# askerlee/segtran

Hardware: AMD Instinct MI355X
Metric: train-step images/sec (cfg2, re-associated op order) (higher is better)
Workload: dtype f32; 1 GPU; REFUGE fundus 2D, segtran eff-b4, translayers 3, layercompress 1,1,2,2, 512x512, bs 6/GPU; global_batch=6, per_gpu_batch=6, parallelism=dp1, step=fwd+BCE/Dice+bwd+allreduce+clip+BertAdam, op_order=re-associated, ranks=1

## Files before the change

### include/segx.h

```cpp
#ifndef SEGX_H
#define SEGX_H
#include <stdint.h>
#ifdef __cplusplus
extern "C" {
#endif

int segx_version(void);
int segx_last_error(char* buf, int buflen);

enum { SEGX_EPI_NONE = 0, SEGX_EPI_GELU = 1 ,
       SEGX_EPI_SWISH = 2  };
enum { SEGX_BIAS_NONE = 0, SEGX_BIAS_N = 1 , SEGX_BIAS_M = 2  };
enum { SEGX_ENGINE_F32 = 0, SEGX_ENGINE_BF16X6 = 1 };
enum { SEGX_ENGINE_SEL_DEFAULT = 0, SEGX_ENGINE_SEL_F32 = 1, SEGX_ENGINE_SEL_BF16X6 = 2 };
enum { SEGX_TILE_AUTO = 0, SEGX_TILE_128x128 = 1, SEGX_TILE_64x64 = 2, SEGX_TILE_128x32 = 3, SEGX_TILE_32x128 = 4, SEGX_TILE_64x128 = 5,
       SEGX_TILE_256x128 = 6, SEGX_TILE_WS128x128 = 7, SEGX_TILE_WS128x256 = 8, SEGX_TILE_WS64x256 = 9,
       SEGX_TILE_WS96x256 = 10, SEGX_TILE_WS256x96 = 11,
       SEGX_TILE_SKINNY_NT = 12   };
typedef struct {
    int32_t M, N, K, nb0, nb1;
    int64_t a_b0, a_b1, a_m, a_k;
    int64_t b_b0, b_b1, b_n, b_k;
    int64_t c_b0, c_b1, c_m;
    float alpha;
// ... 74 lines not shown
int segx_seg_loss_fwd(const float* logits, const float* mask, const float* pos_weight, const float* class_w, float* out,
                      float* ws, int B, int C, int64_t S, float dice_w, void* stream);
int segx_seg_loss_bwd(const float* logits, const float* mask, const float* pos_weight, const float* class_w, const float* ws,
                      const float* grad_out, float* dlogits, int B, int C, int64_t S, float dice_w, void* stream);
int segx_mt_bertadam_step(void* const* params, const void* const* grads, void* const* m, void* const* v, const int64_t* sizes,
                          const int* chunk_tensor, const int64_t* chunk_off, const int* chunk_first, const int* active,
                          const float* lr, const float* wd, int ntensors, int nchunks, int chunk,
                          float max_global_norm, float max_tensor_norm, float sched, float b1, float b2, float eps,
                          float* ws, void* stream);

int segx_mt_gather(const void* const* src, void* const* dst, const int64_t* sizes, const int* chunk_tensor, const int64_t* chunk_off,
                   int chunk_begin, int nchunks, int chunk, void* stream);

int64_t segx_bn_ws_floats(int B, int C, int64_t S);
int segx_bn_act_bwd_reduce(const float* dY, const float* X, const float* mean, const float* var, const float* w, const float* b,
                           float* dw, float* db, float* ws, int B, int C, int64_t S, float eps, int act,
                           const float* gate, const float* dpool, float inv_S, float dc_p, uint64_t seed, uint64_t offset, void* stream);
int segx_bn_act_bwd_apply(const float* dY, const float* X, const float* mean, const float* var, const float* w, const float* b,
                          const float* sum_dw, const float* sum_db, float* dX, int B, int C, int64_t S, float eps, int act,
                          float inv_n, const float* gate, const float* dpool, float inv_S, float dc_p, uint64_t seed, uint64_t offset, void* stream);
int64_t segx_plane_chunks(int64_t S);
int64_t segx_bn_pool_chunks(int B, int64_t S, int auto_stats);
int64_t segx_bn_parts_floats(int B, int C, int64_t S);
int segx_bn_stats_local(const float* X, float* part, float* ws, int B, int C, int64_t S, void* stream);
int segx_bn_act_fwd2(const float* X, const float* parts, int nparts, float* mean, float* var, float* run_mean, float* run_var, float momentum,
                     const float* w, const float* b, float* Y, float* psum, const float* resid, float dc_p, uint64_t seed, uint64_t offset,
                     int B, int C, int64_t S, float eps, int act, int64_t parts_floats, int64_t y_bs, void* stream);
int segx_team_status(int clear);
int segx_team_cap(void);
int segx_occupy(int wgs, int heavy, float ms, float* sink, void* stream);
int segx_bn_act_bwd2(const float* dY, const float* X, const float* mean, const float* var, const float* w, const float* b,
                     float* dX, float* dw, float* db, float* ws, int B, int C, int64_t S, float eps, int act, int training,
                     const float* gate, const float* dpool, float inv_S, float dc_p, uint64_t seed, uint64_t offset, int64_t dy_bs, int64_t ws_floats, void* stream);
int segx_se_fwd2(const float* psum, int nch, float inv_S, const float* W1, const float* b1, const float* W2, const float* b2, const float* Wproj,
                 float* p, float* hpre, float* gate, float* Wb, int B, int C, int Cs, int M, void* stream);
int64_t segx_se_ws2_floats(int B, int C, int Cs);
int segx_se_bwd2(const float* dWb, const float* Wproj, const float* dgate, const float* gate, const float* hpre, const float* p, const float* W1,
                 const float* W2, float inv_S, float* dpool, float* dW1, float* db1, float* dW2, float* db2, float* dWproj, float* ws,
                 int B, int C, int Cs, int M, void* stream);
int segx_dwconv2d_fwd(const float* X, const float* W, float* Y, int B, int C, int H, int Wd, int OH, int OW, int k, int stride,
                      int pad_t, int pad_l, void* stream);
int64_t segx_dwconv2d_pool_chunks(int OH, int OW);
int segx_dwconv2d_bias_act_pool(const float* X, const float* W, const float* bias, float* Y, float* psum, int B, int C, int H, int Wd, int OH, int OW,
                                int k, int stride, int pad_t, int pad_l, int act, void* stream);
int segx_dwconv2d_bwd_data(const float* dY, const float* W, float* dX, int B, int C, int H, int Wd, int OH, int OW, int k,
                           int stride, int pad_t, int pad_l, void* stream);
int64_t segx_dwconv2d_wgrad_rows(int OH, int OW);
int64_t segx_dwconv2d_bwd_fused_rows(int H, int Wd, int OH, int OW, int k, int stride, int pad_t, int pad_l);
int segx_dwconv2d_bwd_fused(const float* dY, const float* X, const float* W, float* dX, float* part, int B, int C, int H, int Wd, int OH, int OW,
                            int k, int stride, int pad_t, int pad_l, void* stream);
int segx_dwconv2d_bwd_weight_direct(const float* dY, const float* X, float* dW, int B, int C, int H, int Wd, int OH, int OW, int k,
                                    int stride, int pad_t, int pad_l, void* stream);
int segx_dwconv2d_bwd_weight(const float* dY, const float* X, float* part, int B, int C, int H, int Wd, int OH, int OW, int k,
                             int stride, int pad_t, int pad_l, void* stream);
int segx_plane_scale(const float* X, const float* gate, float* Y, int64_t planes, int64_t S, void* stream);
int segx_plane_bias_add(const float* X, const float* bias, float* Y, int64_t planes, int C, int64_t S, void* stream);
int segx_plane_dot(const float* A, const float* Bm, float* out, int64_t planes, int64_t S, void* stream);

int64_t segx_gn_ws_floats(int B, int C, int G);
int segx_groupnorm_fwd(const float* X, const float* w, const float* b, float* Y, float* mean, float* rstd, float* ws,
                       int B, int C, int G, int64_t S, float eps, void* stream);
int segx_groupnorm_bwd(const float* dY, const float* X, const float* w, const float* mean, const float* rstd, float* dX,
                       float* dw, float* db, float* ws, int B, int C, int G, int64_t S, float* plane_dx_sums, void* stream);
int64_t segx_interp_gn_nparts(int64_t float4_per_plane, int cpg);
int segx_interp_linear_fwd_axis2_gn(const float* in, const float* base, float* out, int64_t outer, int n1_in, int n1_out, int n2_in, int n2_out,
                                    int64_t inner, int cpg, float* parts, int nparts, void* stream);
// ... 117 lines not shown
```

### segtran_amd/csrc/backbone.hip

```cpp
#include "common.h"
#include <mutex>
#include <unordered_map>

namespace segx {

enum { ACT_NONE = 0, ACT_SWISH = 1, ACT_RELU = 2, ACT_LEAKY = 3  };

__device__ __forceinline__ float sigm(float x) { return 1.0f / (1.0f + __expf(-x)); }
__device__ __forceinline__ float act_fwd(float u, int act) {
    return act == ACT_SWISH ? u * sigm(u) : act == ACT_RELU ? fmaxf(u, 0.f) : act == ACT_LEAKY ? (u > 0.f ? u : 0.2f * u) : u;
}
__device__ __forceinline__ float act_grad(float u, int act) {
    if (act == ACT_SWISH) { const float s = sigm(u); return s * (1.0f + u * (1.0f - s)); }
    if (act == ACT_RELU) return u > 0.f ? 1.0f : 0.f;
    if (act == ACT_LEAKY) return u > 0.f ? 1.0f : 0.2f;
    return 1.0f;
}

__device__ __forceinline__ float drop_connect_scale(float p, uint64_t seed, uint64_t offset, const uint64_t* __restrict__ rbase, int sample) {
    if (!(p > 0.f)) return 1.0f;
    return dropout_scale(seed, 0, offset + (rbase ? *rbase : 0) + (uint64_t)sample, p, 1.0f / (1.0f - p));
}
__device__ __forceinline__ void bn_fold_sums(const float* __restrict__ ws, int c, int nparts, float& a, float& q) {
    const int lane = threadIdx.x & 63;
// ... 1313 lines not shown
        float a = 0.f;
#pragma unroll 16
        for (int i = 0; i < n; ++i) a += dz[i] * W2[(int64_t)(k0 + i) * Cs + j];
        part[((int64_t)b * gridDim.x + blockIdx.x) * Cs + j] = a;
    }
}
__global__ __launch_bounds__(256) void se_wgrad_all_kernel(const float* __restrict__ dz2, const float* __restrict__ dhpre, const float* __restrict__ p,
                                                           const float* __restrict__ hpre, float* __restrict__ dW1, float* __restrict__ db1,
                                                           float* __restrict__ dW2, float* __restrict__ db2, const float* __restrict__ dWb,
                                                           const float* __restrict__ gate, float* __restrict__ dW, int B, int C, int Cs, int64_t MK) {
    const int64_t idx = (int64_t)blockIdx.x * 256 + threadIdx.x, n1 = (int64_t)C * Cs;
    if (idx < n1) {
        const int c = (int)(idx / Cs), j = (int)(idx % Cs);
        float a1 = 0.f, a2 = 0.f, s1 = 0.f, s2 = 0.f;
        for (int b = 0; b < B; ++b) {
            const float hp = hpre[(int64_t)b * Cs + j], dz = dz2[(int64_t)b * C + c], dh = dhpre[(int64_t)b * Cs + j];
            a2 += dz * (hp * sigm(hp)); a1 += dh * p[(int64_t)b * C + c]; s2 += dz; s1 += dh;
        }
        dW2[(int64_t)c * Cs + j] = a2; dW1[(int64_t)j * C + c] = a1;
        if (j == 0) db2[c] = s2;
        if (c == 0) db1[j] = s1;
        return;
    }
    const int64_t i = idx - n1;
    if (!dWb || i >= MK) return;
    const int k = (int)(i % C);
    float s = 0.f;
    for (int b = 0; b < B; ++b) s += dWb[(int64_t)b * MK + i] * gate[(int64_t)b * C + k];
    dW[i] = s;
}

static inline int plane_chunks(int64_t S, int per_thread) { return (int)i64max(1, i64min(64, (S + 256 * per_thread - 1) / (256 * per_thread))); }

}

using namespace segx;
#define SEGX_STREAM hipStream_t stream = (hipStream_t)stream_

static inline int64_t bn_team_floats(int B, int C, int64_t S, bool backward) {
    int kp = 0;
    if (S <= 0 || bn_auto_form(B, S, backward, &kp) != 1) return 0;
    return (int64_t)C * B * bn_team_chunks(S, kp) * (TEAM_SLOT + TEAM_MBOX);
}
template <int LDS_FLOATS>
__global__ __launch_bounds__(256) void occupy_kernel(unsigned long long ticks, float* sink) {
    __shared__ float hold[LDS_FLOATS];
    const unsigned long long t0 = wall_clock64();
    float acc = 0.f;
    while (wall_clock64() - t0 < ticks) { acc += hold[threadIdx.x & 15]; __builtin_amdgcn_s_sleep(32); }
    if (sink && acc == 12345.678f) sink[0] = acc;
}
extern "C" int segx_occupy(int wgs, int heavy, float ms, float* sink, void* stream_) {
    SEGX_STREAM; SEGX_REQUIRE(wgs > 0 && wgs <= 65535 && ms >= 0.f && ms <= 2000.f, "segx_occupy: bad args");
    const unsigned long long ticks = (unsigned long long)(ms * 1e5f);
    if (heavy) hipLaunchKernelGGL((occupy_kernel<20 * 1024>), dim3(wgs), dim3(256), 0, stream, ticks, sink);
    else hipLaunchKernelGGL((occupy_kernel<16>), dim3(wgs), dim3(256), 0, stream, ticks, sink);
    return check_launch("segx_occupy");
}
extern "C" int segx_team_status(int clear) {
    const TeamHost& h = team_host();
    const unsigned n = __atomic_load_n(h.host, __ATOMIC_RELAXED);
    if (clear && n) __atomic_fetch_sub(h.host, n, __ATOMIC_RELAXED);
    return (int)(n > 0x7fffffffu ? 0x7fffffffu : n);
}
extern "C" int segx_team_cap(void) { return team_cap(); }
extern "C" int64_t segx_bn_ws_floats(int B, int C, int64_t S) { return i64max((int64_t)B * C * BN_SLABS * 2, bn_team_floats(B, C, S, true)); }
// ... 112 lines not shown
    SEGX_REQUIRE(dy_bs >= (int64_t)C * S && ((S & 3) != 0 || (dy_bs & 3) == 0), "segx_bn_act_bwd2: bad dY batch stride %lld", (long long)dy_bs);
    SEGX_REQUIRE((int64_t)B * C <= 65535 && dc_p >= 0.f && dc_p < 1.f, "segx_bn_act_bwd2: more than 65535 (sample, channel) planes / bad drop_connect rate");
    int tkp = 0;
    const int af = training ? bn_auto_form(B, S, true, &tkp) : 0;
    BnBwdArgs g;
    g.dY = dY; g.X = X; g.mean = mean; g.var = var; g.w = w; g.b = b; g.dX = dX; g.dw = dw; g.db = db; g.gate = gate; g.dpool = dpool; g.inv_S = inv_S;
    g.dc_p = dc_p; g.seed = seed; g.offset = offset; g.rbase = rng_base(); g.C = C; g.S = S; g.eps = eps; g.act = act; g.dy_bs = dy_bs;
    if (af == 1) {
        BnTeam t; t.B = B; t.cpp = bn_team_chunks(S, tkp); t.slots = ws; t.mbox = ws + (int64_t)C * B * t.cpp * TEAM_SLOT;
        team_fill(t);
        SEGX_REQUIRE(B * t.cpp <= team_cap() && (int64_t)C * B * t.cpp < 2147483647LL, "segx_bn_act_bwd2: team of %d workgroups", B * t.cpp);
        const dim3 tg = team_grid((int64_t)C * B * t.cpp);
        if (tkp == 4) return bn_team_launch_bwd<4>(g, t, tg, stream);
        if (tkp == 8) return bn_team_launch_bwd<8>(g, t, tg, stream);
        return bn_team_launch_bwd<16>(g, t, tg, stream);
    }
    const int form = af == 2 ? bn_res_form(B, S, true) : 0;
    if (form) {
        const int team = form >> 4, kp = form & 15;
        const dim3 rgrid(team == 64 ? (C + 3) / 4 : C);
        if (team == 64) bn_res_launch_bwd<64, 1, 8>(g, B, rgrid, stream);
        else if (kp == 1 && B <= 6) bn_res_launch_bwd<256, 1, 6>(g, B, rgrid, stream);
        else if (kp == 1) bn_res_launch_bwd<256, 1, 8>(g, B, rgrid, stream);
        else if (kp == 2) bn_res_launch_bwd<256, 2, 8>(g, B, rgrid, stream);
        else return fail(-1, "segx_bn_act_bwd2: no resident form %d", form);
        return check_launch("segx_bn_act_bwd2/resident");
    }
    const int nsl = bn_slabs(S);
    hipLaunchKernelGGL(bn_act_bwd_stage1, dim3(C, B, nsl), dim3(256), 0, stream, dY, X, mean, var, w, b, ws, C, S, eps, act, gate, dpool, inv_S, dc_p, seed, offset, rng_base(), dy_bs);
    const float inv_n = training ? 1.0f / ((float)B * (float)S) : 0.f;
    hipLaunchKernelGGL((bn_act_bwd_apply<true>), dim3(plane_chunks(S, 8), B * C), dim3(256), 0, stream, dY, X, mean, var, w, b, (const float*)nullptr,
                       (const float*)nullptr, dX, C, S, eps, act, inv_n, gate, dpool, inv_S, dc_p, seed, offset, rng_base(), (const float*)ws, B * nsl, dw, db, dy_bs);
    return check_launch("segx_bn_act_bwd2");
}
extern "C" int segx_se_fwd2(const float* psum, int nch, float inv_S, const float* W1, const float* b1, const float* W2, const float* b2, const float* Wproj,
                            float* p, float* hpre, float* gate, float* Wb, int B, int C, int Cs, int M, void* stream_) {
    SEGX_STREAM; SEGX_REQUIRE(psum && nch > 0 && W1 && b1 && W2 && b2 && p && hpre && gate && B > 0 && C > 0 && Cs > 0 && (!Wproj || (Wb && M > 0)), "segx_se_fwd2: bad args");
    SEGX_REQUIRE(C <= SE_MAX_C && Cs <= SE_MAX_CS && B <= 65535, "segx_se_fwd2: C=%d / Cs=%d exceed %d / %d", C, Cs, SE_MAX_C, SE_MAX_CS);
    hipLaunchKernelGGL(se_hidden2_kernel, dim3((Cs + 3) / 4, B), dim3(256), 0, stream, psum, nch, inv_S, W1, b1, p, hpre, C, Cs);
    hipLaunchKernelGGL(se_gate_weights_kernel, dim3((C + SE2_CHUNK - 1) / SE2_CHUNK, B, Wproj ? (M + SE2_ROWS - 1) / SE2_ROWS : 1), dim3(256), 0, stream, (const float*)hpre, W2, b2, Wproj, gate, Wb, C, Cs, M);
    return check_launch("segx_se_fwd2");
}
extern "C" int64_t segx_se_ws2_floats(int B, int C, int Cs) { return (int64_t)B * (C + Cs) + (int64_t)B * ((C + SE2_CHUNK - 1) / SE2_CHUNK) * Cs; }
extern "C" int segx_se_bwd2(const float* dWb, const float* Wproj, const float* dgate, const float* gate, const float* hpre, const float* p, const float* W1,
                            const float* W2, float inv_S, float* dpool, float* dW1, float* db1, float* dW2, float* db2, float* dWproj, float* ws,
                            int B, int C, int Cs, int M, void* stream_) {
    SEGX_STREAM; SEGX_REQUIRE(gate && hpre && p && W1 && W2 && dpool && dW1 && db1 && dW2 && db2 && ws && B > 0 && C > 0 && Cs > 0, "segx_se_bwd2: bad args");
    SEGX_REQUIRE((dWb && Wproj && dWproj && M > 0) || (!dWb && !Wproj && dgate), "segx_se_bwd2: either (dWb, Wproj, dWproj, M) or dgate");
    SEGX_REQUIRE(C <= SE_MAX_C && Cs <= SE_MAX_CS && B <= 65535, "segx_se_bwd2: C=%d / Cs=%d exceed %d / %d", C, Cs, SE_MAX_C, SE_MAX_CS);
    const int nchunks = (C + SE2_CHUNK - 1) / SE2_CHUNK;
    float* dz2 = ws; float* dhpre = ws + (int64_t)B * C; float* part = dhpre + (int64_t)B * Cs;
    hipLaunchKernelGGL(se_bwd_gate_kernel, dim3(nchunks, B), dim3(256), 0, stream, dWb, Wproj, dgate, gate, W2, dz2, part, M, C, Cs);
    hipLaunchKernelGGL(se_bwd_pool_kernel, dim3((C + 255) / 256, B), dim3(256), 0, stream, (const float*)part, hpre, W1, inv_S, dhpre, dpool, C, Cs, nchunks);
    const int64_t MK = dWb ? (int64_t)M * C : 0, total = (int64_t)C * Cs + MK;
    hipLaunchKernelGGL(se_wgrad_all_kernel, dim3((unsigned)((total + 255) / 256)), dim3(256), 0, stream, (const float*)dz2, (const float*)dhpre, p, hpre,
                       dW1, db1, dW2, db2, dWb, gate, dWproj, B, C, Cs, MK);
    return check_launch("segx_se_bwd2");
}

#define SEGX_DW_DISPATCH(KERNEL, ...)                                                                          \
    if (k == 3 && stride == 1) hipLaunchKernelGGL((KERNEL<3, 1>), grid, dim3(256), 0, stream, __VA_ARGS__);     \
    else if (k == 3 && stride == 2) hipLaunchKernelGGL((KERNEL<3, 2>), grid, dim3(256), 0, stream, __VA_ARGS__); \
    else if (k == 5 && stride == 1) hipLaunchKernelGGL((KERNEL<5, 1>), grid, dim3(256), 0, stream, __VA_ARGS__); \
    else if (k == 5 && stride == 2) hipLaunchKernelGGL((KERNEL<5, 2>), grid, dim3(256), 0, stream, __VA_ARGS__); \
    else return segx::fail(-1, "depthwise conv: kernel %d stride %d unsupported (k in {3,5}, stride in {1,2})", k, stride);
#define SEGX_DW_ROWS_DISPATCH(FLIP, ...)                                                                                          \
// ... 201 lines not shown
```

### segtran_amd/efficientnet/model.py

```python
import math
import torch
from torch import nn
from torch.nn import functional as F

from .. import functional as SF

BN_MOM, BN_EPS = 1 - 0.99, 1e-3

_BASE = [(1, 3, 1, 1, 32, 16, 0.25), (2, 3, 2, 6, 16, 24, 0.25), (2, 5, 2, 6, 24, 40, 0.25), (3, 3, 2, 6, 40, 80, 0.25),
         (3, 5, 1, 6, 80, 112, 0.25), (4, 5, 2, 6, 112, 192, 0.25), (1, 3, 1, 6, 192, 320, 0.25)]
_PARAMS = {'efficientnet-b0': (1.0, 1.0, 224, 0.2), 'efficientnet-b1': (1.0, 1.1, 240, 0.2),
           'efficientnet-b2': (1.1, 1.2, 260, 0.3), 'efficientnet-b3': (1.2, 1.4, 300, 0.3),
           'efficientnet-b4': (1.4, 1.8, 380, 0.4), 'efficientnet-b5': (1.6, 2.2, 456, 0.4),
           'efficientnet-b6': (1.8, 2.6, 528, 0.5), 'efficientnet-b7': (2.0, 3.1, 600, 0.5)}


def round_filters(filters, width, divisor=8):
    filters *= width
    new = max(divisor, int(filters + divisor / 2) // divisor * divisor)
    if new < 0.9 * filters:
        new += divisor
    return int(new)


# ... 29 lines not shown

def drop_connect(x, p, training):
    if not training:
        return x
    keep = 1 - p
    r = keep + torch.rand([x.shape[0], 1, 1, 1], dtype=x.dtype, device=x.device)
    return x / keep * torch.floor(r)


def fold_conv_bn(weight, bn):
    with torch.no_grad():
        s = bn.weight.double() / torch.sqrt(bn.running_var.double() + bn.eps)
        w = (weight.double() * s.view(-1, *([1] * (weight.dim() - 1)))).float().contiguous()
        b = (bn.bias.double() - bn.running_mean.double() * s).float().contiguous()
    return w, b


class MBConvBlock(nn.Module):
    def __init__(self, k, s, e, cin, cout, se_ratio, image_size):
        super().__init__()
        self.stride, self.expand_ratio, self.input_filters, self.output_filters = s, e, cin, cout
        oup = cin * e
        if e != 1:
            self._expand_conv = Conv2dStaticSamePadding(cin, oup, 1, image_size=image_size, bias=False)
            self._bn0 = nn.BatchNorm2d(oup, momentum=BN_MOM, eps=BN_EPS)
        self._depthwise_conv = Conv2dStaticSamePadding(oup, oup, k, stride=s, image_size=image_size, groups=oup, bias=False)
        self._bn1 = nn.BatchNorm2d(oup, momentum=BN_MOM, eps=BN_EPS)
        nsq = max(1, int(cin * se_ratio))
        self._se_reduce = Conv2dStaticSamePadding(oup, nsq, 1, image_size=1)
        self._se_expand = Conv2dStaticSamePadding(nsq, oup, 1, image_size=1)
        self._project_conv = Conv2dStaticSamePadding(oup, cout, 1, image_size=math.ceil(image_size / s), bias=False)
        self._bn2 = nn.BatchNorm2d(cout, momentum=BN_MOM, eps=BN_EPS)

    gate_in_weights = True

    def folded_operands(self):
        f0 = fold_conv_bn(self._expand_conv.weight, self._bn0) if self.expand_ratio != 1 else None
        return f0, fold_conv_bn(self._depthwise_conv.weight, self._bn1), fold_conv_bn(self._project_conv.weight, self._bn2)

    def forward_folded(self, inputs, folded):
        f0, (w1, b1), (w2, b2) = folded
        x = inputs
        skip = self.stride == 1 and self.input_filters == self.output_filters
        if f0 is not None:
            x = SF.conv1x1(x, f0[0], f0[1], act=SF.ACT_SWISH)
        dw = self._depthwise_conv
        y, psum, nch = SF.dwconv2d_bias_act_pool(x, w1, b1, dw.stride[0], dw.static_pad, SF.ACT_SWISH)
        Wb = SF.se_gate_weights(y, psum, nch, self._se_reduce.weight, self._se_reduce.bias, self._se_expand.weight, self._se_expand.bias, w2)
        return SF.conv1x1_per_sample_bias(y, Wb, b2, resid=inputs if skip else None)

    def forward(self, inputs, drop_connect_rate=None):
        x = skip_in = inputs
        skip = self.stride == 1 and self.input_filters == self.output_filters
        if self.expand_ratio != 1:
            x = SF.bn_act(self._expand_conv(x), self._bn0, SF.ACT_SWISH)
        se = (self._se_reduce.weight, self._se_reduce.bias, self._se_expand.weight, self._se_expand.bias)
        rate = float(drop_connect_rate) if (skip and drop_connect_rate and self.training) else 0.0
        if MBConvBlock.gate_in_weights:
            y, Wb = SF.bn_act_gate_weights(self._depthwise_conv(x), self._bn1, SF.ACT_SWISH, *se, self._project_conv.weight)
            x = SF.conv1x1_per_sample(y, Wb)
        else:
            x = self._project_conv(SF.bn_act_se(self._depthwise_conv(x), self._bn1, SF.ACT_SWISH, *se))
        return SF.bn_act(x, self._bn2, SF.ACT_NONE, resid=skip_in if skip else None, drop_connect=rate)


class EfficientNet(nn.Module):
    def __init__(self, model_name='efficientnet-b4', stem_stride=2, drop_connect_rate=0.2, num_classes=1000):
        super().__init__()
        width, depth, res, _ = _PARAMS[model_name]
        self.drop_connect_rate = drop_connect_rate
        self.stem_stride = stem_stride
        c0 = round_filters(32, width)
        self._conv_stem = Conv2dStaticSamePadding(3, c0, 3, stride=stem_stride, image_size=res, bias=False)
        self._bn0 = nn.BatchNorm2d(c0, momentum=BN_MOM, eps=BN_EPS)
        size = math.ceil(res / 2)
        self._blocks = nn.ModuleList([])
        self.endpoint_seg_indices = [0, 1, 2, 4]
        self.endpoint_blk_indices = []
        for i, (r, k, s, e, cin, cout, se) in enumerate(_BASE):
            cin, cout, r = round_filters(cin, width), round_filters(cout, width), round_repeats(r, depth)
            self._blocks.append(MBConvBlock(k, s, e, cin, cout, se, size))
            size = math.ceil(size / s)
            for _ in range(r - 1):
                self._blocks.append(MBConvBlock(k, 1, e, cout, cout, se, size))
            if i in self.endpoint_seg_indices:
                self.endpoint_blk_indices.append(len(self._blocks))
        chead = round_filters(1280, width)
        self._conv_head = Conv2dStaticSamePadding(cout, chead, 1, image_size=size, bias=False)
# ... 120 lines not shown
```

### segtran_amd/functional.py

```python
import math
import torch
import torch.nn.functional as F
from . import segx
from .segx import EPI_NONE, EPI_GELU, EPI_SWISH, BIAS_NONE, BIAS_N, BIAS_M

LN_EPS = 1e-12


_MRO = torch.autograd.Function.__mro__
_fast_apply = torch._C._FunctionBase in _MRO and not any('apply' in c.__dict__ for c in _MRO[1:_MRO.index(torch._C._FunctionBase)])


class _Fn(torch.autograd.Function):

    @classmethod
    def apply(cls, *args):
        if _fast_apply and not torch._C._are_functorch_transforms_active():
            return super(torch.autograd.Function, cls).apply(*args)
        return super().apply(*args)


def _live(t):
    return t.requires_grad and torch.is_grad_enabled()

# ... 779 lines not shown
    return _BNActCat.apply(head, training, act, *flat)


_bn_ticks = None


def defer_bn_ticks():
    global _bn_ticks
    if _bn_ticks is None:
        _bn_ticks = []


def flush_bn_ticks():
    global _bn_ticks
    ticks, _bn_ticks = _bn_ticks, None
    if ticks:
        torch._foreach_add_(ticks, 1)


def _bn_tick(bn):
    if bn.training and bn.num_batches_tracked is not None:
        if _bn_ticks is not None:
            _bn_ticks.append(bn.num_batches_tracked)
        else:
            bn.num_batches_tracked.add_(1)


def bn_act(x, bn, act=ACT_NONE, resid=None, drop_connect=0.0):
    _bn_tick(bn)
    return _BNAct.apply(x, bn.weight, bn.bias, bn.running_mean, bn.running_var, bn.training, float(bn.momentum), float(bn.eps), act, resid,
                        float(drop_connect or 0.0))


def bn_act_multi(x, bns, act=ACT_NONE):
    mom, eps, training = float(bns[0].momentum), float(bns[0].eps), bns[0].training
    assert all(float(b.momentum) == mom and float(b.eps) == eps and b.training == training for b in bns)
    w, b = torch.cat([m.weight for m in bns]), torch.cat([m.bias for m in bns])
    rm, rv = torch.cat([m.running_mean for m in bns]), torch.cat([m.running_var for m in bns])
    y = _BNAct.apply(x, w, b, rm, rv, training, mom, eps, act, None, 0.0)
    if training:
        sizes = [m.num_features for m in bns]
        with torch.no_grad():
            torch._foreach_copy_([m.running_mean for m in bns] + [m.running_var for m in bns], list(rm.split(sizes)) + list(rv.split(sizes)))
        for m in bns:
            if m.num_batches_tracked is not None:
                if _bn_ticks is not None:
                    _bn_ticks.append(m.num_batches_tracked)
                else:
                    m.num_batches_tracked.add_(1)
    return y


class _DWConv(_Fn):
    fused_backward = True

    @staticmethod
    def forward(ctx, x, w, stride, pad):
        L = segx.lib()
        x, w = _c(x), _c(w)
        B, C, H, W = x.shape
        k = w.shape[-1]
        pl, pr, pt, pb = pad
        OH, OW = (H + pt + pb - k) // stride + 1, (W + pl + pr - k) // stride + 1
        y = _empty(x, B, C, OH, OW)
        L.dwconv2d_fwd(x, w, y, B, C, H, W, OH, OW, k, stride, pt, pl)
        ctx.cfg = (B, C, H, W, OH, OW, k, stride, pt, pl)
# ... 1175 lines not shown
```

### segtran_amd/segx.py

```python
import contextlib
import ctypes
import enum
import os
import torch

_HERE = os.path.dirname(os.path.abspath(__file__))
LIB_PATH = os.path.join(_HERE, 'lib', 'libsegx.so')

c_f = ctypes.c_float
c_i = ctypes.c_int32
c_l = ctypes.c_int64
c_u = ctypes.c_uint64
c_p = ctypes.c_void_p


class GemmDesc(ctypes.Structure):
    _fields_ = [('M', c_i), ('N', c_i), ('K', c_i), ('nb0', c_i), ('nb1', c_i),
                ('a_b0', c_l), ('a_b1', c_l), ('a_m', c_l), ('a_k', c_l),
                ('b_b0', c_l), ('b_b1', c_l), ('b_n', c_l), ('b_k', c_l),
                ('c_b0', c_l), ('c_b1', c_l), ('c_m', c_l),
                ('alpha', c_f), ('epilogue', c_i), ('bias_mode', c_i), ('bias_b1', c_l),
                ('bias', c_p), ('aux', c_p), ('gmax', c_p),
                ('dropout_p', c_f), ('seed', c_u), ('offset', c_u),
                ('splitk', c_i), ('workspace', c_p), ('tile', c_i), ('bias_b0', c_l), ('batch_reduce', c_i), ('engine', c_i),
# ... 287 lines not shown
    def modes_aggr_bwd_all(self, dY, Z, lnw, lnb, wa, stats, dZ, dscore, dlnw, dlnb, dwa, ws, Mo, R, F, p, seed, offset):
        self._call('segx_modes_aggr_bwd_all', Z, dY, Z, lnw, lnb, wa, stats, dZ, dscore, dlnw, dlnb, dwa, ws, Mo, R, F, p, seed, offset)

    def gelu_bwd_colsum_ws(self, rows, N):
        return int(self.c.segx_gelu_bwd_colsum_ws_floats(rows, N))

    def gelu_bwd_colsum(self, dH, T, dT, colsum, ws, rows, N, p, seed, offset):
        self._call('segx_gelu_bwd_colsum', dH, dH, T, dT, colsum, ws, rows, N, p, seed, offset)

    def gelu_bwd(self, dH, T, dT, n, p, seed, offset):
        self._call('segx_gelu_bwd', T, dH, T, dT, n, p, seed, offset)

    def loss_ws(self, B, C):
        return int(self.c.segx_loss_ws_floats(B, C))

    def seg_loss_fwd(self, logits, mask, pw, cw, out, ws, B, C, S, dice_w):
        self._call('segx_seg_loss_fwd', logits, logits, mask, pw, cw, out, ws, B, C, S, dice_w)

    def seg_loss_bwd(self, logits, mask, pw, cw, ws, gout, dlogits, B, C, S, dice_w):
        self._call('segx_seg_loss_bwd', logits, logits, mask, pw, cw, ws, gout, dlogits, B, C, S, dice_w)

    def bn_ws(self, B, C, S=0):
        return int(self.c.segx_bn_ws_floats(B, C, S))

    def plane_chunks(self, S):
        return int(self.c.segx_plane_chunks(S))

    def bn_pool_chunks(self, B, S, auto_stats):
        return int(self.c.segx_bn_pool_chunks(B, S, 1 if auto_stats else 0))

    def bn_parts_floats(self, B, C, S=0):
        return int(self.c.segx_bn_parts_floats(B, C, S))

    def bn_stats_local(self, X, part, ws, B, C, S):
        self._call('segx_bn_stats_local', X, X, part, ws, B, C, S)

    def bn_act_fwd2(self, X, parts, nparts, mean, var, run_mean, run_var, momentum, w, b, Y, psum, resid, dc_p, seed, offset, B, C, S, eps, act, y_bs=0):
        if y_bs:
            self._chk_t(Y)
            assert Y.device == X.device and Y.dtype == torch.float32 and Y.stride(1) == S and Y.stride(0) == y_bs and Y[0].is_contiguous()
            Y = Y.data_ptr()
        self._call('segx_bn_act_fwd2', X, X, parts, nparts, mean, var, run_mean, run_var, momentum, w, b, Y, psum, resid, float(dc_p), seed, offset, B, C, S, eps, act,
                   0 if parts is None else parts.numel(), int(y_bs))

    def bn_act_bwd2(self, dY, X, mean, var, w, b, dX, dw, db, ws, B, C, S, eps, act, training, gate=None, dpool=None, inv_S=0.0, dc_p=0.0, seed=0, offset=0, dy_bs=0):
        self._chk_t(dY, X, mean, var, w, b, dX, dw, db, ws, gate, dpool)
        for t in (X, mean, var, w, b, dX, dw, db, ws):
            assert t.is_contiguous()
        assert dy_bs or dY.is_contiguous()
        rc = self.c.segx_bn_act_bwd2(_ptr(dY), _ptr(X), _ptr(mean), _ptr(var), _ptr(w), _ptr(b), _ptr(dX), _ptr(dw), _ptr(db), _ptr(ws), B, C, S, eps, act, training,
                                     _ptr(gate), _ptr(dpool), float(inv_S), float(dc_p), seed, offset, int(dy_bs), ws.numel(), self.stream(X))
        self.check(rc, 'segx_bn_act_bwd2')

    def se_fwd2(self, psum, nch, inv_S, W1, b1, W2, b2, Wproj, p, hpre, gate, Wb, B, C, Cs, M):
        self._call('segx_se_fwd2', gate, psum, nch, inv_S, W1, b1, W2, b2, Wproj, p, hpre, gate, Wb, B, C, Cs, M)

    def se_ws2(self, B, C, Cs):
        return int(self.c.segx_se_ws2_floats(B, C, Cs))

    def se_bwd2(self, dWb, Wproj, dgate, gate, hpre, p, W1, W2, inv_S, dpool, dW1, db1, dW2, db2, dWproj, ws, B, C, Cs, M):
        self._call('segx_se_bwd2', gate, dWb, Wproj, dgate, gate, hpre, p, W1, W2, inv_S, dpool, dW1, db1, dW2, db2, dWproj, ws, B, C, Cs, M)

    def dwconv2d_fwd(self, X, W, Y, B, C, H, Wd, OH, OW, k, stride, pt, pl):
        self._call('segx_dwconv2d_fwd', X, X, W, Y, B, C, H, Wd, OH, OW, k, stride, pt, pl)

    def dwconv2d_pool_chunks(self, OH, OW):
# ... 305 lines not shown
    'segx_posbias_fwd': 'ppplipffpp', 'segx_posbias_bwd': 'pppplipffp',
    'segx_softmax_fwd': 'ppplifpfuup', 'segx_softmax_bwd': 'pppplifpfuup',
    'segx_layernorm_fwd': 'pppppplifp', 'segx_layernorm_bwd': 'pppppplip',
    'segx_colreduce_ws_floats': 'lli', 'segx_colsum': 'pppllp', 'segx_ln_param_grad': 'ppppppplip',
    'segx_sum': 'plppfp', 'segx_rowsum': 'ppllp',
    'segx_prenorm_fwd': 'pppplfpppliiffuup',
    'segx_prenorm_bwd': 'ppppplfppppliifuup',
    'segx_prenorm_bwd_all_ws_floats': 'ii', 'segx_prenorm_bwd_all': 'ppppplfpppppppiiifuup',
    'segx_posembed_fwd': 'pppppliifp', 'segx_posembed_bwd': 'ppppppliip',
    'segx_modes_aggr_fwd': 'pppppppiliffuup', 'segx_modes_aggr_bwd': 'ppppppppilifuup',
    'segx_modes_aggr_param_grad': 'pppppppppppilifuup', 'segx_gelu_bwd': 'ppplfuup',
    'segx_gelu_bwd_colsum': 'ppppplifuup', 'segx_gelu_bwd_colsum_ws_floats': 'li', 'segx_modes_aggr_bwd_all_ws_floats': 'ili', 'segx_modes_aggr_bwd_all': 'ppppppppppppilifuup',
    'segx_loss_ws_floats': 'ii', 'segx_seg_loss_fwd': 'ppppppiilfp', 'segx_seg_loss_bwd': 'pppppppiilfp',
    'segx_mt_bertadam_step': 'pppppppppppiiiffffffpp', 'segx_mt_gather': 'pppppiiip',
    'segx_gn_ws_floats': 'iii', 'segx_groupnorm_fwd': 'pppppppiiilfp', 'segx_groupnorm_bwd': 'pppppppppiiilpp',
    'segx_interp_gn_nparts': 'li', 'segx_interp_linear_fwd_axis2_gn': 'pppliiiilipip', 'segx_groupnorm_fwd_parts': 'ppipppppiiilfp',
    'segx_groupnorm_stats_parts': 'pippifp', 'segx_gn_fold_bwd': 'pppppppppiiilp', 'segx_bridge_mask': 'ppppiiiiiiiiip', 'segx_gn_fold_bwd_proj': 'ppippppppppiiilp',
    'segx_interp_linear_fwd': 'pppliiiiiip', 'segx_interp_linear_fwd_axis2': 'pppliiiilp', 'segx_interp_linear_bwd_axis2': 'ppliiiilp', 'segx_interp_linear_bwd': 'ppliiiiiip', 'segx_interp_linear_bwd_axis': 'ppliilfp',
    'segx_axis_gather': 'pplpp', 'segx_pixel_shuffle2': 'ppliiip', 'segx_add_noise': 'ppplffiuup', 'segx_resize2d': 'ppliiiiiip', 'segx_color_blend': 'ppilippip',
    'segx_gray_mean_ws_floats': 'il', 'segx_gray_mean': 'pppilip', 'segx_normalize': 'ppiilfppp',
    'segx_x6_presplit_elems': 'iiii', 'segx_x6_presplit': 'piilliillpp',
    'segx_tune': 'ii', 'segx_tune_get': 'i', 'segx_x3_launches': '', 'segx_gemm_route': 'pppp', 'segx_set_rng_base': 'p', 'segx_rng_advance': 'pup', 'segx_resized_crop3d': 'pplpp', 'segx_stem_compose_fwd': 'ppppiiiiip', 'segx_stem_compose_bwd': 'pppppppiiiiip', 'segx_bridge_input': 'ppiiiiiip', 'segx_stem_s2d_input': 'ppiiiiiip', 'segx_conv2d_stem_fwd': 'pppiiiiiiiiiiip', 'segx_conv2d_stem_im2col': 'ppiiiiiiiiiiip', 'segx_dropout': 'pplfuup', 'segx_avgpool2_fwd': 'ppliip', 'segx_avgpool2_bwd': 'ppliip', 'segx_transpose': 'ppliip', 'segx_interp_linear_fwd_axis': 'pppliilfp', 'segx_window_accum': 'pppiipp', 'segx_harden_segmap': 'ppppiilifp', 'segx_window_gather': 'ppppiiipp', 'segx_window_merge': 'pppppiiipifp', 'segx_dice_ws_floats': 'll', 'segx_dice_sums': 'pppllp',
    'segx_conv3d_fwd': 'pppiipipp', 'segx_conv3d_fwd_packed': 'pppiipipp', 'segx_conv3d_fwd_packed_bs': 'pppiipipllp', 'segx_conv3d_bwd_weight_packed_bs': 'pppiipipllp', 'segx_conv3d_pack_weights': 'ppiiiip', 'segx_conv3d_splitk': 'iipi', 'segx_conv3d_route': 'iipiiiip', 'segx_conv3d_fwd_terms': 'iipiii', 'segx_conv3d_flip_weights': 'ppiiip', 'segx_conv3d_bwd_weight': 'pppiipipp', 'segx_conv3d_bwd_weight_packed': 'pppiipipp', 'segx_conv3d_unpack_wgrad': 'ppiiip',
    'segx_conv3d_halo_ok': 'iip', 'segx_conv3d_halo_wq_floats': 'ii', 'segx_conv3d_halo_pack': 'ppiiip', 'segx_conv3d_halo_fwd': 'pppiipllip', 'segx_conv3d_halo_wgrad_ok': 'iip', 'segx_conv3d_halo_wgrad_ws_floats': 'iip', 'segx_conv3d_halo_wgrad': 'ppppiipllp',
    'segx_conv3d_bwd_data_direct': 'ppppiipp', 'segx_nonzero_mask': 'ppiiiiiiiip', 'segx_label_nhot': 'ppiilip',
    'segx_maxpool3d_fwd': 'ppplpp', 'segx_maxpool3d_bwd': 'ppplppp',
    'segx_bn_ws_floats': 'iil', 
    'segx_dwconv2d_fwd': 'pppiiiiiiiiiip', 'segx_dwconv2d_bwd_data': 'pppiiiiiiiiiip',
    'segx_dwconv2d_pool_chunks': 'ii', 'segx_dwconv2d_bias_act_pool': 'pppppiiiiiiiiiiip', 'segx_conv2d_stem_bias_act_fwd': 'ppppiiiiiiiiiiiip',
    'segx_dwconv2d_bwd_weight': 'pppiiiiiiiiiip', 'segx_dwconv2d_bwd_weight_direct': 'pppiiiiiiiiiip', 'segx_dwconv2d_wgrad_rows': 'ii', 'segx_dwconv2d_bwd_fused_rows': 'iiiiiiii', 'segx_dwconv2d_bwd_fused': 'pppppiiiiiiiiiip', 'segx_plane_scale': 'pppllp', 'segx_plane_dot': 'pppllp',
     'segx_plane_bias_add': 'ppplilp', 
    'segx_plane_chunks': 'l', 'segx_bn_pool_chunks': 'ili', 'segx_bn_parts_floats': 'iil', 'segx_bn_stats_local': 'pppiilp',
    'segx_bn_act_fwd2': 'ppippppfpppppfuuiilfillp', 'segx_bn_act_bwd2': 'ppppppppppiilfiippffuullp',
    'segx_team_status': 'i', 'segx_team_cap': '', 'segx_occupy': 'iifpp',
    'segx_se_fwd2': 'pifpppppppppiiiip', 'segx_se_ws2_floats': 'iii', 'segx_se_bwd2': 'ppppppppfpppppppiiiip',
    'segx_bn_act_bwd_reduce': 'pppppppppiilfippffuup', 'segx_bn_act_bwd_apply': 'pppppppppiilfifppffuup',
}

_LIB = None
DEFAULT_ENGINE = 'x6'


def lib():
    global _LIB
    if _LIB is None:
        _LIB = SegxLib(LIB_PATH)
        _LIB.set_engine(os.environ.get('SEGX_ENGINE', DEFAULT_ENGINE))
    return _LIB


def use_library(libobj):
    global _LIB
    _LIB = libobj
```

Baseline: 92.25 images/s.

## Fuse expand 1x1 conv with BN+swish via input second-moment statistics

For MBConv expand convs with small input channel count (<=32), BN batch statistics are computed from the input's mean and covariance (mean = W·mu, var = W^T Σ W) instead of from the materialized conv output. A single apply kernel then recomputes the 1x1 conv per pixel and writes both the pre-activation and the swish output. This avoids writing and re-reading the wide expanded tensor for the stats pass. The cost is double-precision moment accumulation and variance computed through a covariance formula, which can lose precision relative to direct two-pass stats.

```diff
diff --git a/include/segx.h b/include/segx.h
--- a/include/segx.h
+++ b/include/segx.h
@@ -130,6 +130,12 @@
 int segx_bn_act_bwd2(const float* dY, const float* X, const float* mean, const float* var, const float* w, const float* b,
                      float* dX, float* dw, float* db, float* ws, int B, int C, int64_t S, float eps, int act, int training,
                      const float* gate, const float* dpool, float inv_S, float dc_p, uint64_t seed, uint64_t offset, int64_t dy_bs, int64_t ws_floats, void* stream);
+int64_t segx_expand_moments_floats(int B, int K, int64_t S);
+int segx_expand_moments(const float* X, float* ws, int64_t ws_floats, int B, int K, int64_t S, void* stream);
+int segx_expand_bn_finalize(const float* ws, const float* W, const float* gamma, const float* beta, float* mean, float* var, float* scale, float* shift,
+                            float* run_mean, float* run_var, float momentum, float eps, int B, int K, int C, int64_t S, void* stream);
+int segx_expand_bn_act_apply(const float* X, const float* W, const float* scale, const float* shift, float* pre, float* act, int B, int K, int C, int64_t S,
+                             void* stream);
 int segx_se_fwd2(const float* psum, int nch, float inv_S, const float* W1, const float* b1, const float* W2, const float* b2, const float* Wproj,
                  float* p, float* hpre, float* gate, float* Wb, int B, int C, int Cs, int M, void* stream);
 int64_t segx_se_ws2_floats(int B, int C, int Cs);
diff --git a/segtran_amd/csrc/backbone.hip b/segtran_amd/csrc/backbone.hip
--- a/segtran_amd/csrc/backbone.hip
+++ b/segtran_amd/csrc/backbone.hip
@@ -1369,6 +1369,199 @@
 
 static inline int plane_chunks(int64_t S, int per_thread) { return (int)i64max(1, i64min(64, (S + 256 * per_thread - 1) / (256 * per_thread))); }
 
+constexpr int EXM_KMAX = 56, EXM_TP = 128, EXM_LD = EXM_TP + 1;
+static inline int exm_k4(int K) { return (K + 3) / 4; }
+static inline int exm_nb(int K) { return exm_k4(K) * (exm_k4(K) + 1) / 2; }
+static inline int exm_pw(int K) { return exm_nb(K) * 16 + exm_k4(K) * 4; }
+static inline int64_t exm_tiles(int64_t S) { return (S + EXM_TP - 1) / EXM_TP; }
+static inline int exm_chunks(int B, int K, int64_t S) { return (int)i64max(1, i64min(exm_tiles(S), (K <= 32 ? 1024 : 512) / B)); }
+static inline int64_t exm_head(int K) { return (int64_t)K + (int64_t)K * K; }
+__device__ __forceinline__ void exm_block(int blk, int K4, int& bi, int& bj) {
+    if (blk < K4) { bi = bj = blk; return; }
+    int rem = blk - K4; bi = 0;
+    while (rem >= K4 - 1 - bi) { rem -= K4 - 1 - bi; ++bi; }
+    bj = bi + 1 + rem;
+}
+
+__global__ __launch_bounds__(256) void expand_moments_kernel(const float* __restrict__ X, double* __restrict__ part, int K, int64_t S, int tiles_per_wg) {
+    __shared__ float xs[EXM_KMAX * EXM_LD];
+    __shared__ double red[256 * 4];
+    const int t = threadIdx.x, K4 = (K + 3) / 4, NB = K4 * (K4 + 1) / 2, nsl = 256 / NB;
+    const int blk = t / nsl, sl = t % nsl;
+    const bool live = blk < NB, diag = blk < K4;
+    int bi = 0, bj = 0;
+    if (live) exm_block(blk, K4, bi, bj);
+    const int b = blockIdx.y;
+    const int64_t ntiles = (S + EXM_TP - 1) / EXM_TP, tile0 = (int64_t)blockIdx.x * tiles_per_wg;
+    const int64_t tile1 = tile0 + tiles_per_wg < ntiles ? tile0 + tiles_per_wg : ntiles;
+    double acc[16], sx[4];
+#pragma unroll
+    for (int e = 0; e < 16; ++e) acc[e] = 0.0;
+#pragma unroll
+    for (int r = 0; r < 4; ++r) sx[r] = 0.0;
+    for (int64_t tile = tile0; tile < tile1; ++tile) {
+        const int64_t p0 = tile * EXM_TP;
+        for (int idx = t; idx < K4 * 4 * (EXM_TP / 4); idx += 256) {
+            const int r = idx / (EXM_TP / 4), q = idx % (EXM_TP / 4);
+            const int64_t p = p0 + q * 4;
+            float4 v = make_float4(0.f, 0.f, 0.f, 0.f);
+            if (r < K && p < S) v = *reinterpret_cast<const float4*>(X + ((int64_t)b * K + r) * S + p);
+            float* d = xs + r * EXM_LD + q * 4;
+            d[0] = v.x; d[1] = v.y; d[2] = v.z; d[3] = v.w;
+        }
+        __syncthreads();
+        if (live) {
+            const float* xa = xs + bi * 4 * EXM_LD; const float* xb = xs + bj * 4 * EXM_LD;
+            for (int p = sl; p < EXM_TP; p += nsl) {
+                double a[4], c[4];
+#pragma unroll
+                for (int r = 0; r < 4; ++r) { a[r] = (double)xa[r * EXM_LD + p]; c[r] = (double)xb[r * EXM_LD + p]; }
+#pragma unroll
+                for (int r = 0; r < 4; ++r) {
+#pragma unroll
+                    for (int q = 0; q < 4; ++q) acc[r * 4 + q] = fma(a[r], c[q], acc[r * 4 + q]);
+                }
+                if (diag) {
+#pragma unroll
+                    for (int r = 0; r < 4; ++r) sx[r] += a[r];
+                }
+            }
+        }
+        __syncthreads();
+    }
+    double* out = part + ((int64_t)blockIdx.y * gridDim.x + blockIdx.x) * (NB * 16 + K4 * 4);
+#pragma unroll
+    for (int round = 0; round < 5; ++round) {
+#pragma unroll
+        for (int r = 0; r < 4; ++r) red[t * 4 + r] = round < 4 ? acc[round * 4 + r] : sx[r];
+        __syncthreads();
+        if (live && sl == 0 && (round < 4 || diag)) {
+            double s[4];
+#pragma unroll
+            for (int r = 0; r < 4; ++r) s[r] = red[t * 4 + r];
+            for (int o = 1; o < nsl; ++o) {
+#pragma unroll
+                for (int r = 0; r < 4; ++r) s[r] += red[(t + o) * 4 + r];
+            }
+#pragma unroll
+            for (int r = 0; r < 4; ++r) out[round < 4 ? blk * 16 + round * 4 + r : NB * 16 + bi * 4 + r] = s[r];
+        }
+        __syncthreads();
+    }
+}
+__global__ __launch_bounds__(256) void expand_moments_reduce_kernel(const double* __restrict__ part, double* __restrict__ head, int K, int nwg) {
+    __shared__ double red[256];
+    const int t = threadIdx.x, K4 = (K + 3) / 4, NB = K4 * (K4 + 1) / 2, PW = NB * 16 + K4 * 4;
+    const int e = blockIdx.x * 8 + (t & 7), run = t >> 3;
+    double s = 0.0;
+    if (e < PW) for (int w = run; w < nwg; w += 32) s += part[(int64_t)w * PW + e];
+    red[t] = s;
+    __syncthreads();
+    if (run != 0 || e >= PW) return;
+    for (int o = 1; o < 32; ++o) s += red[o * 8 + t];
+    if (e >= NB * 16) {
+        const int i = e - NB * 16;
+        if (i < K) head[i] = s;
+        return;
+    }
+    int bi, bj;
+    exm_block(e >> 4, K4, bi, bj);
+    const int i = bi * 4 + ((e >> 2) & 3), j = bj * 4 + (e & 3);
+    if (i >= K || j >= K) return;
+    head[K + i * K + j] = s;
+    if (bi != bj) head[K + j * K + i] = s;
+}
+__global__ __launch_bounds__(256) void expand_bn_finalize_kernel(const double* __restrict__ head, const float* __restrict__ W, const float* __restrict__ gamma,
+                                                                 const float* __restrict__ beta, float* __restrict__ mean, float* __restrict__ var, float* __restrict__ scale,
+                                                                 float* __restrict__ shift, float* __restrict__ run_mean, float* __restrict__ run_var, float momentum,
+                                                                 float eps, int K, int C, double n) {
+    __shared__ double cov[EXM_KMAX * (EXM_KMAX + 1)];
+    __shared__ double mv[EXM_KMAX];
+    const int t = threadIdx.x, lane = t & 63, w = t >> 6, KS = K | 1;
+    const double inv_n = 1.0 / n;
+    for (int idx = t; idx < K * K; idx += 256) {
+        const int i = idx / K, j = idx % K;
+        cov[i * KS + j] = head[K + idx] * inv_n - (head[i] * inv_n) * (head[j] * inv_n);
+    }
+    if (t < K) mv[t] = head[t] * inv_n;
+    __syncthreads();
+    const int c = blockIdx.x * 4 + w;
+    double q = 0.0, m = 0.0;
+    if (c < C && lane < K) {
+        const float* wc = W + (int64_t)c * K;
+        const double* row = cov + lane * KS;
+        double a[4] = {0.0, 0.0, 0.0, 0.0};
+        int j = 0;
+        for (; j + 4 <= K; j += 4) {
+#pragma unroll
+            for (int u = 0; u < 4; ++u) a[u] = fma(row[j + u], (double)wc[j + u], a[u]);
+        }
+        for (; j < K; ++j) a[0] = fma(row[j], (double)wc[j], a[0]);
+        q = (double)wc[lane] * ((a[0] + a[1]) + (a[2] + a[3])); m = (double)wc[lane] * mv[lane];
+    }
+#pragma unroll
+    for (int o = 32; o > 0; o >>= 1) { q += __shfl_xor(q, o); m += __shfl_xor(m, o); }
+    if (c >= C || lane != 0) return;
+    if (!(q > 0.0)) q = 0.0;
+    const float mf = (float)m, vf = (float)q;
+    mean[c] = mf; var[c] = vf;
+    const float sc = rsqrtf(vf + eps) * gamma[c];
+    scale[c] = sc; shift[c] = beta[c] - mf * sc;
+    if (run_mean) {
+        run_mean[c] = (1.0f - momentum) * run_mean[c] + momentum * mf;
+        run_var[c] = (1.0f - momentum) * run_var[c] + momentum * (float)(q * (n / (n > 2.0 ? n - 1.0 : 1.0)));
+    }
+}
+template <int PT> struct ExpVec { typedef float4 type; };
+template <> struct ExpVec<2> { typedef float2 type; };
+__device__ __forceinline__ void exp_unpack(const float4& v, float (&o)[4]) { o[0] = v.x; o[1] = v.y; o[2] = v.z; o[3] = v.w; }
+__device__ __forceinline__ void exp_unpack(const float2& v, float (&o)[2]) { o[0] = v.x; o[1] = v.y; }
+__device__ __forceinline__ float4 exp_pack(const float (&o)[4]) { return make_float4(o[0], o[1], o[2], o[3]); }
+__device__ __forceinline__ float2 exp_pack(const float (&o)[2]) { return make_float2(o[0], o[1]); }
+template <int KP, int PT, bool EXACT>
+__device__ __forceinline__ void expand_apply_body(const float* __restrict__ X, const float* __restrict__ W, const float* __restrict__ scale, const float* __restrict__ shift,
+                                                  float* __restrict__ pre, float* __restrict__ act, int K, int C, int64_t S, int c0, int c1, int b, int64_t p) {
+    typedef typename ExpVec<PT>::type V;
+    float x[KP][PT];
+    const float* xp = X + (int64_t)b * K * S + p;
+#pragma unroll
+    for (int k = 0; k < KP; ++k) {
+        if (EXACT || k < K) exp_unpack(*reinterpret_cast<const V*>(xp + (int64_t)k * S), x[k]);
+        else {
+#pragma unroll
+            for (int j = 0; j < PT; ++j) x[k][j] = 0.f;
+        }
+    }
+    int64_t o = ((int64_t)b * C + c0) * S + p;
+    for (int c = c0; c < c1; ++c, o += S) {
+        const float* wc = W + (int64_t)c * K;
+        float a[PT], y[PT];
+#pragma unroll
+        for (int j = 0; j < PT; ++j) a[j] = 0.f;
+#pragma unroll
+        for (int k = 0; k < KP; ++k) {
+            const float wk = wc[EXACT ? k : (k < K ? k : K - 1)];
+#pragma unroll
+            for (int j = 0; j < PT; ++j) a[j] = fmaf(x[k][j], wk, a[j]);
+        }
+        const float sc = scale[c], sh = shift[c];
+#pragma unroll
+        for (int j = 0; j < PT; ++j) y[j] = act_fwd(a[j] * sc + sh, ACT_SWISH);
+        *reinterpret_cast<V*>(pre + o) = exp_pack(a);
+        *reinterpret_cast<V*>(act + o) = exp_pack(y);
+    }
+}
+template <int KP, int PT>
+__global__ __launch_bounds__(256) void expand_bn_act_apply_kernel(const float* __restrict__ X, const float* __restrict__ W, const float* __restrict__ scale,
+                                                                  const float* __restrict__ shift, float* __restrict__ pre, float* __restrict__ act, int K, int C,
+                                                                  int64_t S, int cper) {
+    const int64_t p = ((int64_t)blockIdx.x * 256 + threadIdx.x) * PT;
+    if (p >= S) return;
+    const int c0 = blockIdx.z * cper, c1 = c0 + cper < C ? c0 + cper : C, b = blockIdx.y;
+    if (K == KP) expand_apply_body<KP, PT, true>(X, W, scale, shift, pre, act, K, C, S, c0, c1, b, p);
+    else expand_apply_body<KP, PT, false>(X, W, scale, shift, pre, act, K, C, S, c0, c1, b, p);
+}
+
 }
 
 using namespace segx;
@@ -1547,6 +1740,55 @@
     hipLaunchKernelGGL((bn_act_bwd_apply<true>), dim3(plane_chunks(S, 8), B * C), dim3(256), 0, stream, dY, X, mean, var, w, b, (const float*)nullptr,
                        (const float*)nullptr, dX, C, S, eps, act, inv_n, gate, dpool, inv_S, dc_p, seed, offset, rng_base(), (const float*)ws, B * nsl, dw, db, dy_bs);
     return check_launch("segx_bn_act_bwd2");
+}
+extern "C" int64_t segx_expand_moments_floats(int B, int K, int64_t S) {
+    if (B <= 0 || K <= 0 || K > EXM_KMAX || S <= 0) return 0;
+    return 2 * (exm_head(K) + (int64_t)B * exm_chunks(B, K, S) * exm_pw(K));
+}
+extern "C" int segx_expand_moments(const float* X, float* ws, int64_t ws_floats, int B, int K, int64_t S, void* stream_) {
+    SEGX_STREAM; SEGX_REQUIRE(X && ws && B > 0 && B <= 65535 && K > 0 && K <= EXM_KMAX && S > 0 && (S & 3) == 0, "segx_expand_moments: bad args (1 <= K <= %d, S %% 4 == 0)", EXM_KMAX);
+    SEGX_REQUIRE((reinterpret_cast<uintptr_t>(X) & 15) == 0 && (reinterpret_cast<uintptr_t>(ws) & 7) == 0, "segx_expand_moments: X needs 16-byte, the workspace 8-byte alignment");
+    const int64_t need = segx_expand_moments_floats(B, K, S);
+    SEGX_REQUIRE(ws_floats >= need, "segx_expand_moments: the workspace holds %lld floats, this call needs %lld (segx_expand_moments_floats)", (long long)ws_floats, (long long)need);
+    const int tiles_per_wg = (int)((exm_tiles(S) + exm_chunks(B, K, S) - 1) / exm_chunks(B, K, S)), chunks = (int)((exm_tiles(S) + tiles_per_wg - 1) / tiles_per_wg);
+    double* head = reinterpret_cast<double*>(ws); double* part = head + exm_head(K);
+    hipLaunchKernelGGL(expand_moments_kernel, dim3(chunks, B), dim3(256), 0, stream, X, part, K, S, tiles_per_wg);
+    hipLaunchKernelGGL(expand_moments_reduce_kernel, dim3((exm_pw(K) + 7) / 8), dim3(256), 0, stream, (const double*)part, head, K, B * chunks);
+    return check_launch("segx_expand_moments");
+}
+extern "C" int segx_expand_bn_finalize(const float* ws, const float* W, const float* gamma, const float* beta, float* mean, float* var, float* scale, float* shift,
+                                       float* run_mean, float* run_var, float momentum, float eps, int B, int K, int C, int64_t S, void* stream_) {
+    SEGX_STREAM; SEGX_REQUIRE(ws && W && gamma && beta && mean && var && scale && shift && (!run_mean == !run_var) && B > 0 && K > 0 && K <= EXM_KMAX && C > 0 && S > 0,
+                              "segx_expand_bn_finalize: bad args");
+    SEGX_REQUIRE((reinterpret_cast<uintptr_t>(ws) & 7) == 0, "segx_expand_bn_finalize: the workspace needs 8-byte alignment");
+    hipLaunchKernelGGL(expand_bn_finalize_kernel, dim3((C + 3) / 4), dim3(256), 0, stream, reinterpret_cast<const double*>(ws), W, gamma, beta, mean, var, scale, shift,
+                       run_mean, run_var, momentum, eps, K, C, (double)B * (double)S);
+    return check_launch("segx_expand_bn_finalize");
+}
+template <int KP, int PT>
+static void expand_apply_launch(const float* X, const float* W, const float* scale, const float* shift, float* pre, float* act, int B, int K, int C, int64_t S, hipStream_t stream) {
+    const int64_t gx = (S + 256 * PT - 1) / (256 * PT);
+    int split = 1;
+    while (gx * B * split < 1024 && split < 32 && (C + 2 * split - 1) / (2 * split) >= 16) split *= 2;
+    const int cper = (C + split - 1) / split;
+    hipLaunchKernelGGL((expand_bn_act_apply_kernel<KP, PT>), dim3((unsigned)gx, B, (C + cper - 1) / cper), dim3(256), 0, stream, X, W, scale, shift, pre, act, K, C, S, cper);
+}
+extern "C" int segx_expand_bn_act_apply(const float* X, const float* W, const float* scale, const float* shift, float* pre, float* act, int B, int K, int C, int64_t S,
+                                        void* stream_) {
+    SEGX_STREAM; SEGX_REQUIRE(X && W && scale && shift && pre && act && B > 0 && B <= 65535 && K > 0 && K <= EXM_KMAX && C > 0 && S > 0 && (S & 3) == 0,
+                              "segx_expand_bn_act_apply: bad args (1 <= K <= %d, S %% 4 == 0)", EXM_KMAX);
+    SEGX_REQUIRE(((reinterpret_cast<uintptr_t>(X) | reinterpret_cast<uintptr_t>(pre) | reinterpret_cast<uintptr_t>(act)) & 15) == 0 && S / 512 < 2147483647LL,
+                 "segx_expand_bn_act_apply: X, pre and act need 16-byte alignment");
+    switch ((K + 7) / 8) {
+    case 1: expand_apply_launch<8, 4>(X, W, scale, shift, pre, act, B, K, C, S, stream); break;
+    case 2: expand_apply_launch<16, 4>(X, W, scale, shift, pre, act, B, K, C, S, stream); break;
+    case 3: expand_apply_launch<24, 4>(X, W, scale, shift, pre, act, B, K, C, S, stream); break;
+    case 4: expand_apply_launch<32, 2>(X, W, scale, shift, pre, act, B, K, C, S, stream); break;
+    case 5: expand_apply_launch<40, 2>(X, W, scale, shift, pre, act, B, K, C, S, stream); break;
+    case 6: expand_apply_launch<48, 2>(X, W, scale, shift, pre, act, B, K, C, S, stream); break;
+    default: expand_apply_launch<56, 2>(X, W, scale, shift, pre, act, B, K, C, S, stream); break;
+    }
+    return check_launch("segx_expand_bn_act_apply");
 }
 extern "C" int segx_se_fwd2(const float* psum, int nch, float inv_S, const float* W1, const float* b1, const float* W2, const float* b2, const float* Wproj,
                             float* p, float* hpre, float* gate, float* Wb, int B, int C, int Cs, int M, void* stream_) {
diff --git a/segtran_amd/efficientnet/model.py b/segtran_amd/efficientnet/model.py
--- a/segtran_amd/efficientnet/model.py
+++ b/segtran_amd/efficientnet/model.py
@@ -85,6 +85,7 @@
         self._project_conv = Conv2dStaticSamePadding(oup, cout, 1, image_size=math.ceil(image_size / s), bias=False)
         self._bn2 = nn.BatchNorm2d(cout, momentum=BN_MOM, eps=BN_EPS)
 
+    fused_expand = True
     gate_in_weights = True
 
     def folded_operands(self):
@@ -106,7 +107,7 @@
         x = skip_in = inputs
         skip = self.stride == 1 and self.input_filters == self.output_filters
         if self.expand_ratio != 1:
-            x = SF.bn_act(self._expand_conv(x), self._bn0, SF.ACT_SWISH)
+            x = SF.expand_bn_act(x, self._expand_conv.weight, self._bn0, bias=self._expand_conv.bias, fused=MBConvBlock.fused_expand)
         se = (self._se_reduce.weight, self._se_reduce.bias, self._se_expand.weight, self._se_expand.bias)
         rate = float(drop_connect_rate) if (skip and drop_connect_rate and self.training) else 0.0
         if MBConvBlock.gate_in_weights:
diff --git a/segtran_amd/functional.py b/segtran_amd/functional.py
--- a/segtran_amd/functional.py
+++ b/segtran_amd/functional.py
@@ -835,6 +835,52 @@
                         float(drop_connect or 0.0))
 
 
+EXPAND_KERNEL_MAX_CIN = 56
+EXPAND_FUSED_MAX_CIN = 32
+
+
+class _ExpandBNAct(_Fn):
+
+    @staticmethod
+    def forward(ctx, x, W, gamma, beta, run_mean, run_var, momentum, eps):
+        L = segx.lib()
+        B, K = x.shape[0], x.shape[1]
+        C = W.shape[0]
+        S = x.numel() // (B * K)
+        W = _c(W)
+        ws = _empty(x, L.expand_moments_floats(B, K, S))
+        L.expand_moments(x, ws, B, K, S)
+        stats = _empty(x, 4, C)
+        mean, var, scale, shift = stats[0], stats[1], stats[2], stats[3]
+        L.expand_bn_finalize(ws, W, gamma, beta, mean, var, scale, shift, run_mean, run_var, momentum, eps, B, K, C, S)
+        pre = _empty(x, B, C, *x.shape[2:])
+        act = torch.empty_like(pre)
+        L.expand_bn_act_apply(x, W, scale, shift, pre, act, B, K, C, S)
+        ctx.cfg = (B, C, S, eps, ACT_SWISH, True, B * S)
+        ctx.spec = GemmSpec(C, S, K, (0, 0, K, 1), (K * S, 0, 1, S), (C * S, 0, S), tuple(pre.shape), nb=(B, 1), bias_mode=BIAS_M)
+        ctx.save_for_backward(x, W, pre, mean, var, gamma, beta)
+        return act
+
+    @staticmethod
+    def backward(ctx, dy):
+        L = segx.lib()
+        x, W, pre, mean, var, gamma, beta = ctx.saved_tensors
+        dpre, dg, db = _bn_act_backward(L, dy, pre, mean, var, gamma, beta, ctx.cfg)
+        dW = _grad_operand(L, dpre, x, ctx.spec, 'a', W) if ctx.needs_input_grad[1] else None
+        dx = _grad_operand(L, dpre, W, ctx.spec, 'b', x) if ctx.needs_input_grad[0] else None
+        return dx, dW, dg, db, None, None, None, None
+
+
+def expand_bn_act(x, weight, bn, bias=None, fused=True):
+    B, Cin = x.shape[0], x.shape[1]
+    S = x.numel() // max(B * Cin, 1)
+    if (not fused or not bn.training or _bn_stats_sync is not None or bias is not None or Cin > min(EXPAND_FUSED_MAX_CIN, EXPAND_KERNEL_MAX_CIN) or S % 4 != 0 or S == 0
+            or not x.is_contiguous() or bn.running_mean is None):
+        return bn_act(conv1x1(x, weight, bias), bn, ACT_SWISH)
+    _bn_tick(bn)
+    return _ExpandBNAct.apply(x, weight.reshape(weight.shape[0], Cin), bn.weight, bn.bias, bn.running_mean, bn.running_var, float(bn.momentum), float(bn.eps))
+
+
 def bn_act_multi(x, bns, act=ACT_NONE):
     mom, eps, training = float(bns[0].momentum), float(bns[0].eps), bns[0].training
     assert all(float(b.momentum) == mom and float(b.eps) == eps and b.training == training for b in bns)
diff --git a/segtran_amd/segx.py b/segtran_amd/segx.py
--- a/segtran_amd/segx.py
+++ b/segtran_amd/segx.py
@@ -343,6 +343,18 @@
     def bn_parts_floats(self, B, C, S=0):
         return int(self.c.segx_bn_parts_floats(B, C, S))
 
+    def expand_moments_floats(self, B, K, S):
+        return int(self.c.segx_expand_moments_floats(B, K, S))
+
+    def expand_moments(self, X, ws, B, K, S):
+        self._call('segx_expand_moments', X, X, ws, ws.numel(), B, K, S)
+
+    def expand_bn_finalize(self, ws, W, gamma, beta, mean, var, scale, shift, run_mean, run_var, momentum, eps, B, K, C, S):
+        self._call('segx_expand_bn_finalize', ws, ws, W, gamma, beta, mean, var, scale, shift, run_mean, run_var, float(momentum), float(eps), B, K, C, S)
+
+    def expand_bn_act_apply(self, X, W, scale, shift, pre, act, B, K, C, S):
+        self._call('segx_expand_bn_act_apply', X, X, W, scale, shift, pre, act, B, K, C, S)
+
     def bn_stats_local(self, X, part, ws, B, C, S):
         self._call('segx_bn_stats_local', X, X, part, ws, B, C, S)
 
@@ -714,6 +726,7 @@
      'segx_plane_bias_add': 'ppplilp', 
     'segx_plane_chunks': 'l', 'segx_bn_pool_chunks': 'ili', 'segx_bn_parts_floats': 'iil', 'segx_bn_stats_local': 'pppiilp',
     'segx_bn_act_fwd2': 'ppippppfpppppfuuiilfillp', 'segx_bn_act_bwd2': 'ppppppppppiilfiippffuullp',
+    'segx_expand_moments_floats': 'iil', 'segx_expand_moments': 'ppliilp', 'segx_expand_bn_finalize': 'ppppppppppffiiilp', 'segx_expand_bn_act_apply': 'ppppppiiilp',
     'segx_team_status': 'i', 'segx_team_cap': '', 'segx_occupy': 'iifpp',
     'segx_se_fwd2': 'pifpppppppppiiiip', 'segx_se_ws2_floats': 'iii', 'segx_se_bwd2': 'ppppppppfpppppppiiiip',
     'segx_bn_act_bwd_reduce': 'pppppppppiilfippffuup', 'segx_bn_act_bwd_apply': 'pppppppppiilfifppffuup',
```

Result: no change. 92.61 images/s, median of 6 (+0.4%).
